# SeonghwanSeo/PharmacoNet

Hardware: AMD Instinct MI355X
Metric: ligand-conformers scored/sec (1 pocket) (higher is better)
Workload: dtype f32; 1 GPU; 6OIM-like model (37 nodes, 11 clusters) vs 1003520 synthetic ligands per GPU = 4096 molecule topologies x 245 copies with every node displaced (sigma 0.35 A) and every conformer coordinate jittered (sigma 0.30 A); mean 17.1 pharmacophore nodes (<= 32), 8 conformers each, 10 % drawn on the model's nodes; top-1000; library=expanded, pockets=1, ligands_per_gpu=1003520, conformers_per_ligand=8, parallelism=single GPU

## Files before the change

### include/pmx.h

```cpp
#ifndef PMX_H
#define PMX_H

#include <stdint.h>

#ifdef __cplusplus
extern "C" {
#endif

#define PMX_NUM_TYPES 7
#define PMX_MAX_LEVELS 20
#define PMX_MAX_MODEL_NODES 256
#define PMX_MAX_MODEL_CLUSTERS 128
#define PMX_MAX_LEVEL_CANDIDATES 64
#define PMX_MAX_LIGAND_NODES 64
#define PMX_MAX_LIGAND_CLUSTERS 64
#define PMX_MAX_CONFORMERS 64

typedef enum {
    PMX_OK = 0,
    PMX_ERR_INVALID = 1,
    PMX_ERR_HIP = 2,
    PMX_ERR_OOM = 3
} pmx_status;

// ... 73 lines not shown
    const uint64_t *atom_off;
    const uint8_t *atomic_num;
    const uint64_t *nbr_off;
    const int32_t *nbr;
    const uint64_t *feat_off;
    const uint8_t *feat_type;
    const uint8_t *feat_flags;
    const uint64_t *feat_atom_off;
    const int32_t *feat_atoms;
    const uint64_t *feat_center_off;
    const int32_t *feat_centers;
    const int32_t *n_conf;
    const uint64_t *pos_off;
    const float *positions;
} pmx_feature_batch;
int pmx_pack_features(const pmx_feature_batch *batch, int threads, uint64_t *offsets_out, uint8_t *data_out, uint64_t data_cap,
                      uint64_t *data_bytes, int32_t *status_out);
int pmx_pack_features_device(const pmx_feature_batch *batch, int device, void *stream, uint64_t *offsets_out, uint8_t *data_out,
                             uint64_t data_cap, uint64_t *data_bytes, int32_t *status_out);

int pmx_library_select(const pmx_library *lib, const uint64_t *indices_dev, uint64_t n, uint64_t *offsets_out_dev ,
                       uint8_t *data_out_dev, uint64_t data_cap, uint64_t *data_bytes, void *stream);
int pmx_library_buffers(const pmx_library *lib, const uint64_t **offsets_dev, const uint8_t **data_dev);

typedef struct {
    uint64_t n_mols;
    const uint64_t *atom_off;
    const uint8_t *atomic_num;
    const uint8_t *explicit_degree;
    const uint8_t *heavy_degree;
    const uint8_t *hyb;
    const uint8_t *h_count;
    const uint8_t *flags;
    const uint64_t *nbr_off;
    const int32_t *nbr;
    const uint64_t *ring_off;
    const uint64_t *ring_atom_off;
    const int32_t *ring_atoms;
} pmx_atom_batch;
int pmx_perceive_features(const pmx_atom_batch *batch, int threads, uint64_t *feat_off, uint8_t *feat_type, uint8_t *feat_flags,
                          uint64_t *feat_atom_off, int32_t *feat_atoms, uint64_t *feat_center_off, int32_t *feat_centers,
                          uint64_t cap_features, uint64_t cap_atoms, uint64_t cap_centers, uint64_t *n_features, uint64_t *n_feat_atoms,
                          uint64_t *n_feat_centers, int32_t *status_out);

int pmx_sdf_heavy_atoms(const char *text, uint64_t len, uint64_t max_records, uint64_t cap_records, uint64_t cap_atoms,
                        uint64_t *n_records, uint64_t *n_atoms, int32_t *atoms_per_record, uint8_t *atomic_num, float *xyz);
// ... 90 lines not shown
```

### pharmaconet_amd/_ffi.py

```python

from __future__ import annotations

import ctypes
from pathlib import Path

PKG = Path(__file__).resolve().parent
LIB_PATH = PKG / "libpmx.so"

NUM_TYPES = 7
COMM_ID_BYTES = 128


class PmxError(RuntimeError):
    pass


class ModelDesc(ctypes.Structure):
    _fields_ = [
        ("n_nodes", ctypes.c_int32),
        ("n_clusters", ctypes.c_int32),
        ("node_type", ctypes.c_void_p),
        ("edge_mean", ctypes.c_void_p),
        ("edge_std", ctypes.c_void_p),
        ("cluster_nodes", ctypes.c_void_p),
# ... 67 lines not shown

class MatchConstraint(ctypes.Structure):

    _fields_ = [
        ("n_require", ctypes.c_int32),
        ("require", (ctypes.c_uint64 * 2) * MAX_REQUIRE_GROUPS),
        ("exclude", ctypes.c_uint64 * 2),
    ]


SIGNATURES = {
    "pmx_last_error": (ctypes.c_char_p, []),
    "pmx_version": (ctypes.c_int, []),
    "pmx_model_create": (ctypes.c_int, [ctypes.POINTER(ModelDesc), ctypes.c_int, ctypes.POINTER(ctypes.c_void_p)]),
    "pmx_model_destroy": (ctypes.c_int, [ctypes.c_void_p]),
    "pmx_library_upload": (ctypes.c_int, [ctypes.POINTER(LibraryView), ctypes.c_int, ctypes.POINTER(ctypes.c_void_p)]),
    "pmx_library_info_get": (ctypes.c_int, [ctypes.c_void_p, ctypes.POINTER(LibraryInfo)]),
    "pmx_library_destroy": (ctypes.c_int, [ctypes.c_void_p]),
    "pmx_library_select": (
        ctypes.c_int,
        [ctypes.c_void_p, ctypes.c_void_p, ctypes.c_uint64, ctypes.c_void_p, ctypes.c_void_p, ctypes.c_uint64, ctypes.POINTER(ctypes.c_uint64), ctypes.c_void_p],
    ),
    "pmx_library_buffers": (ctypes.c_int, [ctypes.c_void_p, ctypes.POINTER(ctypes.c_void_p), ctypes.POINTER(ctypes.c_void_p)]),
    "pmx_score": (
        ctypes.c_int,
        [ctypes.c_void_p, ctypes.c_void_p, ctypes.POINTER(ctypes.c_float), ctypes.c_uint64, ctypes.c_uint64,
         ctypes.c_void_p, ctypes.c_void_p, ctypes.c_void_p],
    ),
    "pmx_score_multi": (
        ctypes.c_int,
        [ctypes.POINTER(ctypes.c_void_p), ctypes.c_int, ctypes.c_void_p, ctypes.POINTER(ctypes.c_float),
         ctypes.c_uint64, ctypes.c_uint64, ctypes.c_void_p, ctypes.c_void_p, ctypes.c_void_p],
    ),
    "pmx_score_f64": (
        ctypes.c_int,
        [ctypes.c_void_p, ctypes.c_void_p, ctypes.POINTER(ctypes.c_float), ctypes.c_uint64, ctypes.c_uint64,
         ctypes.c_void_p, ctypes.c_void_p, ctypes.c_void_p],
    ),
    "pmx_score_multi_f64": (
        ctypes.c_int,
        [ctypes.POINTER(ctypes.c_void_p), ctypes.c_int, ctypes.c_void_p, ctypes.POINTER(ctypes.c_float),
         ctypes.c_uint64, ctypes.c_uint64, ctypes.c_void_p, ctypes.c_void_p, ctypes.c_void_p],
    ),
    "pmx_topk": (
        ctypes.c_int,
        [ctypes.c_void_p, ctypes.c_void_p, ctypes.c_uint64, ctypes.c_uint64, ctypes.c_int, ctypes.c_void_p,
# ... 133 lines not shown
```

### pharmaconet_amd/build.py

```python

from __future__ import annotations

import os
import shutil
import subprocess
import sys
from pathlib import Path

PKG = Path(__file__).resolve().parent
REPO = PKG.parent
CSRC = PKG / "csrc"
LIB = PKG / "libpmx.so"
PACK_LIB = PKG / "libpmx_pack.so"
SOURCES = ("pmx_api.hip", "pmx_screen_debug.hip", "pmx_explain.hip", "pmx_rows.hip", "pmx_fingerprint.hip", "pmx_topk.hip", "pmx_density.hip", "pmx_pack_device.hip", "pmx_select.hip", "pmx_pack.cpp", "pmx_sdf.cpp", "pmx_perceive.cpp")
DEPS = ("pmx_screen.hip", "pmx_screen_walk.h", "pmx_screen_tables.h", "pmx_screen_layout.h", "pmx_device.h", "pmx_debug.h", "pmx_explain.h", "pmx_rows.h", "pmx_scan.h")
FLAGS = (
    "--offload-arch=gfx950",
    "-O3",
    "-std=c++17",
    "-fPIC",
    "-ffp-contract=off",
    "-fno-fast-math",
    "-Wall",
    "-Wno-unused-function",
    "-mllvm", "-simplifycfg-sink-common=false",
    "-mllvm", "-disable-lsr",
    "-mllvm", "-greedy-regclass-priority-trumps-globalness",
    "-mllvm", "-phi-node-folding-threshold=1",
)


def hipcc() -> str:
    for cand in (os.environ.get("HIPCC"), shutil.which("hipcc"), "/opt/rocm/bin/hipcc"):
        if cand and Path(cand).exists():
            return cand
    raise RuntimeError("hipcc not found")


# ... 97 lines not shown
```

### pharmaconet_amd/csrc/pmx_api.hip

```cpp
#include <hip/hip_runtime.h>

#include <algorithm>
#include <cmath>
#include <cstdarg>
#include <cstdio>
#include <cstdlib>
#include <chrono>
#include <cstring>
#include <cstddef>
#include <memory>
#include <map>
#include <mutex>
#include <string>
#include <thread>
#include <utility>
#include <vector>
#include <time.h>

#include "pmx.h"
#include "pmx_screen.hip"
#include "pmx_debug.h"
#include "pmx_explain.h"
#include "pmx_rows.h"

using namespace pmx;

static thread_local char g_err[512] = "";
static thread_local pmx_score_stats g_stats = {};
static int g_profiling = 0;
struct ScreenWs;
static thread_local std::shared_ptr<ScreenWs> g_last_screen;
static thread_local int g_last_device = 0;
static int screen_stats(pmx_score_stats *out);

static int fail(int code, const char *fmt, ...) {
    va_list ap;
    va_start(ap, fmt);
    vsnprintf(g_err, sizeof(g_err), fmt, ap);
    va_end(ap);
    return code;
}

#define HIPCHECK(expr)                                                                                         \
    do {                                                                                                       \
        hipError_t e_ = (expr);                                                                                \
// ... 456 lines not shown
    lib->info.n_bytes = nbytes;
    lib->info.total_conformers = stats[0];
    lib->info.max_nodes = (int32_t)stats[1];
    lib->info.max_conformers = (int32_t)stats[2];
    lib->info.max_clusters = (int32_t)stats[3];
    lib->info.n_unsupported = (int32_t)stats[4];
    *out = lib;
    return PMX_OK;
}

extern "C" int pmx_library_info_get(const pmx_library *lib, pmx_library_info *info) {
    if (!lib || !info) return fail(PMX_ERR_INVALID, "null argument");
    *info = lib->info;
    return PMX_OK;
}

extern "C" int pmx_library_buffers(const pmx_library *lib, const uint64_t **offsets_dev, const uint8_t **data_dev) {
    if (!lib || !offsets_dev || !data_dev) return fail(PMX_ERR_INVALID, "null argument");
    *offsets_dev = lib->offsets;
    *data_dev = lib->data;
    return PMX_OK;
}

int pmx_library_device(const pmx_library *lib) { return lib->device; }

extern "C" int pmx_library_destroy(pmx_library *lib) {
    if (!lib) return PMX_OK;
    (void)hipSetDevice(lib->device);
    if (lib->owns) (void)hipFree(lib->offsets), (void)hipFree(lib->data);
    delete lib;
    return PMX_OK;
}

static std::mutex g_mu;

static long env_long(const char *name, long dflt) {
    const char *s = std::getenv(name);
    if (!s || !*s) return dflt;
    return std::atol(s);
}

static constexpr size_t kLdsPerCu = 160 * 1024;

static bool trace_on() {
    static int v = -1;
    if (v < 0) v = std::getenv("PMX_TRACE") ? 1 : 0;
    return v == 1;
}

struct ScreenWs {
    DevBuf ctl;
    DevBuf xctl;
    DevBuf slices, big;
    DevBuf totbuf;
    DevBuf pabuf;
    DevBuf arena, queue;
    DevBuf lists;
    DevBuf acur;
    size_t arena_shrunk_to = 0;
    int num_cu = 0;
    hipEvent_t ev[6] = {nullptr, nullptr, nullptr, nullptr, nullptr, nullptr};
    uint64_t ligands_last = 0;
    bool ev_valid = false;
    bool ctl_used = false;
    hipStream_t last_stream = nullptr;
    std::mutex mu;
    uint64_t stamp = 0;
    bool released = false;
    void free_buffers() {
        for (DevBuf *b : {&ctl, &xctl, &slices, &big, &totbuf, &pabuf, &arena, &queue, &lists, &acur}) b->release();
        for (auto &e : ev) {
            if (e) (void)hipEventDestroy(e);
            e = nullptr;
        }
        arena_shrunk_to = 0;
        ev_valid = ctl_used = false;
    }
};
static std::map<std::pair<int, hipStream_t>, std::shared_ptr<ScreenWs>> g_screen;

static uint64_t g_screen_stamp = 0;

static std::shared_ptr<ScreenWs> ensure_screen(int device, hipStream_t stream) {
    std::shared_ptr<ScreenWs> out, victim;
    {
        std::lock_guard<std::mutex> lock(g_mu);
        const auto key = std::make_pair(device, stream);
        auto it = g_screen.find(key);
        if (it != g_screen.end() && it->second) {
            it->second->stamp = ++g_screen_stamp;
            return it->second;
        }
        const long cap = std::max<long>(1, env_long("PMX_MAX_WORKSPACES", 4));
// ... 142 lines not shown
    pl.need.big = (size_t)pl.big_grid * pl.big_bytes;
    if (cand_bounds<G>()) {
        const uint64_t need = (nlmax + 1) * nlmax * K * G * 4;
        p.pa_bytes = (uint32_t)std::min<uint64_t>((need + 255) & ~255ull, (uint64_t)std::max<long>(1, env_long("PMX_PATH_KB", 1024)) << 10);
        pl.need.pabuf = (size_t)grid * p.pa_bytes * 2u;
    }
    if (!totals_in_lds<G>()) pl.need.totbuf = (size_t)num_cu * 4u * std::max(PMX_SCREEN_WAVES, PMX_TASK_WAVES) * kTotBufBytes * 2u;
    if (worst > pl.big_bytes) pl.arena_retries = (int)std::max<long>(1, env_long("PMX_ARENA_RETRIES", 4));
    const long super_dflt = std::max(16384L, (1L << 20) * 8 / std::max(G, 8) / k_scale);
    pl.super = (uint32_t)std::max<long>(1024, std::min<long>(env_long("PMX_SUPER", super_dflt), 1 << 24));
    return PMX_OK;
}

template <int G>
static int score_screen(const pmx_model *const *models, int n_models, const pmx_library *lib, const Weights &W, uint64_t first, uint64_t count,
                        void *scores_dev, bool scores_f64, int32_t *status_dev, hipStream_t stream, ScreenWs &ws) {
    if (count > 0xfffffff0ull) return fail(PMX_ERR_INVALID, "more than 2^32 ligands in one call");
    const uint32_t flags = (uint32_t)env_long("PMX_TREE_FLAGS", 0);
    const uint32_t lig_budget = (uint32_t)std::max<long>(16, env_long("PMX_BUDGET", 768));
    const uint32_t task_budget = (uint32_t)std::max<long>(16, env_long("PMX_TASK_BUDGET", std::min<long>(lig_budget, 384)));
    const int rounds = (int)std::max<long>(1, env_long("PMX_ROUNDS", 12));
    const int task_decay_from = (int)std::max<long>(1, env_long("PMX_TASK_DECAY_FROM", 99));
    const uint32_t task_budget_min = (uint32_t)std::max<long>(8, env_long("PMX_TASK_BUDGET_MIN", 48));
    const bool exact = (flags & 8) != 0;
    const bool debug_kernels = (flags & ~PMX_PRODUCT_FLAGS) != 0;
    bool debug_ok = true;
    const bool tails = pair_tails(models, n_models, W);

    {
        const int irc = init_workspace(ws, lib->device, stream);
        if (irc) return irc;
    }
    std::vector<PocketPlan> plan((size_t)n_models);
    BufferNeeds need;
    uint32_t super_max = 0;
    for (int m = 0; m < n_models; ++m) {
        PocketPlan &pl = plan[(size_t)m];
        const int rc = plan_pocket<G>(models[m], lib, W, ws.num_cu, stream, pl);
        if (rc) return rc;
        ScreenParams &p = pl.p;
        p.first = first;
        p.flags = flags | (scores_f64 ? PMX_SCORES_F64 : 0u);
        p.budget = lig_budget;
        p.min_levels = (uint32_t)std::max<long>(0, env_long("PMX_MIN_LEVELS", 3));
        p.scores = scores_f64 ? reinterpret_cast<float *>(static_cast<double *>(scores_dev) + (size_t)m * count) : static_cast<float *>(scores_dev) + (size_t)m * count;
        p.status = m == 0 ? status_dev : nullptr;
        need.cover(pl.need);
        super_max = std::max(super_max, pl.super);
    }

    {
        int rc = grow_buffers(ws, need, stream);
        if (!rc) rc = ensure_arena<G>(ws, stream);
        if (rc) return rc;
        HIPCHECK(ws.queue.grow((size_t)std::max<long>(1, env_long("PMX_TASKQ_MB", (G >= 32 ? 1024L : 2048L) * std::max(1, G / 8))) << 20, stream));
        HIPCHECK(ws.lists.grow((size_t)super_max * 12, stream));
    }
    Ctl *const ctl = ws.ctl.as<Ctl>();
    uint32_t *const lists = ws.lists.as<uint32_t>();
    uint8_t *const totbuf = ws.totbuf.as<uint8_t>(), *const pabuf = ws.pabuf.as<uint8_t>();

    if (g_profiling) HIPCHECK(hipEventRecord(ws.ev[0], stream));
    ws.ctl_used = false;
    for (int m = 0; m < n_models; ++m) {
        const PocketPlan &pl = plan[(size_t)m];
        ScreenParams p = pl.p;
        const uint32_t super = pl.super;
        const uint32_t lig_grid = (uint32_t)ws.num_cu * pl.waves_per_cu, task_grid = (uint32_t)ws.num_cu * pl.task_waves_per_cu;
        p.ctl = ctl;
        p.arena = ws.arena.as<uint8_t>();
        p.arena_bytes = std::min<unsigned long long>(ws.arena.bytes, (1ull << 36) - 4096);
        p.ovf_list = lists;
        p.carry_list = lists + super;
        p.heavy_list = lists + 2 * (size_t)super;
        p.list_cap = super;
        p.queue = ws.queue.as<uint8_t>();
        p.qcap = (uint32_t)std::min<size_t>(ws.queue.bytes / task_rec_bytes<G>() / kShards, 0x3fffffffu / kShards);
        p.totbuf = totbuf;
        p.pabuf = pabuf;
        auto launch = [&](int mode, uint32_t blocks) {
            p.mode = mode;
            if (debug_kernels) debug_ok &= pmx_debug::launch_ligand(G, exact, tails, blocks, pl.lds, stream, &p, sizeof p);
            else if (tails) ligand_kernel<G, false, true><<<dim3(blocks), dim3(64), pl.lds, stream>>>(p);
            else ligand_kernel<G, false, false><<<dim3(blocks), dim3(64), pl.lds, stream>>>(p);
        };
        auto rounds_and_finalize = [&]() {
            if (!totals_in_lds<G>()) p.totbuf = totbuf + ws.totbuf.bytes / 2;
            if (pabuf) p.pabuf = pabuf + ws.pabuf.bytes / 2;
            for (int r = 0; r < rounds; ++r) {
                p.budget = r < task_decay_from ? task_budget : std::max<uint32_t>(task_budget_min, task_budget >> std::min(r - task_decay_from + 1, 16));
                p.last_round = r + 1 == rounds ? 1u : 0u;
                round_kernel<<<dim3(1), dim3(64), 0, stream>>>(ctl, p.qcap);
                if (debug_kernels) debug_ok &= pmx_debug::launch_task(G, task_grid, pl.lds, stream, &p, sizeof p);
                else task_kernel<G><<<dim3(task_grid), dim3(64), pl.lds, stream>>>(p);
            }
            finalize_kernel<G><<<dim3((super + 255) / 256), dim3(256), 0, stream>>>(p);
            p.last_round = 0;
            p.budget = lig_budget;
            p.totbuf = totbuf;
            p.pabuf = pabuf;
        };
        for (uint64_t lo = 0; lo < count; lo += super) {
            const bool last_of_call = m + 1 == n_models && lo + super >= count;
            p.lo = (uint32_t)lo;
            p.hi = (uint32_t)std::min<uint64_t>(count, lo + super);
            if (g_profiling && last_of_call) HIPCHECK(hipEventRecord(ws.ev[1], stream));
            ws.ligands_last = p.hi - p.lo;
            ctl_clear_kernel<<<dim3((sizeof(Ctl) / 4 + 255) / 256), dim3(256), 0, stream>>>(ctl, ws.ctl_used ? 0 : 1);
            ws.ctl_used = true;
            p.slices = ws.slices.as<uint8_t>();
            p.slice_bytes = pl.slice_bytes;
            launch(0, lig_grid);
            p.slices = ws.big.as<uint8_t>();
            p.slice_bytes = pl.big_bytes;
            launch(1, std::min(pl.big_grid, lig_grid));
            p.retry_out = lists;
            p.retry_slot = 0;
            launch(2, std::min(pl.big_grid, lig_grid));
            if (g_profiling && last_of_call) {
                HIPCHECK(hipEventRecord(ws.ev[2], stream));
                HIPCHECK(hipEventRecord(ws.ev[4], stream));
            }
            rounds_and_finalize();
            for (int t = 0; t < pl.arena_retries; ++t) {
                prepare_retry(p, ctl, lists, super, t, pl.arena_retries, stream);
                launch(3, std::min(pl.big_grid, lig_grid));
                rounds_and_finalize();
            }
// ... 60 lines not shown

static int lanes_of(const pmx_library *lib) {
    int g = 1;
    while (g < std::min(lib->info.max_conformers, PMX_MAX_CONFORMERS)) g <<= 1;
    return g;
}

static Weights to_weights(const float weights[PMX_NUM_TYPES]) {
    Weights W;
    for (int t = 0; t < PMX_NUM_TYPES; ++t) W.w[t] = weights[t];
    return W;
}

struct HeldWs {
    std::shared_ptr<ScreenWs> ws;
    std::unique_lock<std::mutex> lock;
};
static HeldWs hold_screen(int device, hipStream_t stream) {
    for (;;) {
        HeldWs h{ensure_screen(device, stream), {}};
        h.lock = std::unique_lock<std::mutex>(h.ws->mu);
        if (!h.ws->released) return h;
    }
}

static int score_any(const pmx_model *const *models, int n_models, const pmx_library *lib, const float weights[PMX_NUM_TYPES], uint64_t first,
                     uint64_t count, void *scores_dev, bool scores_f64, int32_t *status_dev, void *stream_) {
    if (!models || n_models < 0 || !lib || !weights || (!scores_dev && count && n_models)) return fail(PMX_ERR_INVALID, "null argument");
    for (int i = 0; i < n_models; ++i) {
        if (!models[i]) return fail(PMX_ERR_INVALID, "null model");
        if (models[i]->device != lib->device) return fail(PMX_ERR_INVALID, "model and library live on different devices");
    }
    if (first > lib->info.n_ligands || count > lib->info.n_ligands - first) return fail(PMX_ERR_INVALID, "ligand range out of bounds");
    g_stats = pmx_score_stats{};
    g_last_screen.reset();
    if (count == 0 || n_models == 0) return PMX_OK;
    HIPCHECK(hipSetDevice(lib->device));
    const Weights W = to_weights(weights);
    hipStream_t stream = static_cast<hipStream_t>(stream_);
    const HeldWs held = hold_screen(lib->device, stream);
    int rc = PMX_OK;
    if (!with_lanes(lanes_of(lib), [&](auto g) { rc = score_screen<decltype(g)::value>(models, n_models, lib, W, first, count, scores_dev, scores_f64, status_dev, stream, *held.ws); }))
        rc = fail(PMX_ERR_INVALID, "no kernels for %d conformer lanes", lanes_of(lib));
    g_last_screen = held.ws;
    g_last_device = lib->device;
    return rc;
// ... 234 lines not shown
```

### pharmaconet_amd/csrc/pmx_debug.h

```cpp
#pragma once
#include <hip/hip_runtime.h>
#include <cstddef>

namespace pmx_debug {
bool launch_ligand(int G, bool exact, bool tails, unsigned blocks, unsigned lds, hipStream_t stream, const void *params, size_t bytes);
bool launch_task(int G, unsigned blocks, unsigned lds, hipStream_t stream, const void *params, size_t bytes);
}
```

### pharmaconet_amd/csrc/pmx_screen.hip

```cpp
#include "pmx_screen_walk.h"

#ifndef PMX_SCREEN_WAVES
#define PMX_SCREEN_WAVES 6
#endif
#ifndef PMX_TASK_WAVES
#define PMX_TASK_WAVES 6
#endif

namespace PMX_NS {
using namespace pmx;

template <int G, bool EXACT, bool TAILS>
__global__ __launch_bounds__(64, PMX_SCREEN_WAVES) void ligand_kernel(const ScreenParams p) {
    extern __shared__ __attribute__((aligned(16))) unsigned char lds[];
    const int lane0 = lane_id();
    const uint32_t wave_id = blockIdx.x;
    const WaveShape<G> ws = wave_shape<G>(p.M.K, (int)p.max_nodes);
    const uint32_t todo = p.mode == 0 ? p.hi - p.lo
                          : min(p.mode == 1 ? p.ctl->ovf_count : (p.mode == 2 ? p.ctl->carry_count : p.ctl->retry_count[p.retry_slot ^ 1u]), p.list_cap);
    const uint32_t *list = p.mode == 1 ? p.ovf_list : (p.mode == 2 ? p.carry_list : p.retry_in);
    constexpr uint32_t kBatch = 1;
    WaveStats *stat = reinterpret_cast<WaveStats *>(lds + ws.off_stat);
    if (lane0 < (int)(sizeof(WaveStats) / 8)) reinterpret_cast<unsigned long long *>(stat)[lane0] = 0ull;
    wave_sync();
    const unsigned long long t_start = __builtin_amdgcn_s_memtime();
    uint32_t lig_next = 0, lig_end = 0;
    for (;;) {
        const int lane = lane_id();
        if (lig_next == lig_end) {
            uint32_t base = 0;
            if (lane == 0) base = atomicAdd(&p.ctl->cursor[p.mode], kBatch);
            base = (uint32_t)uni((int)base);
            lig_next = min(base, todo);
            lig_end = min(base + kBatch, todo);
            if (lig_next == lig_end) break;
        }
        const uint32_t next = lig_next++;
        const uint32_t li = p.mode == 0 ? p.lo + next : (uint32_t)uni((int)list[next]);
        unsigned char *rec = prepare_ligand<G, EXACT, TAILS>(p, lds, ws, li, wave_id, stat);
        if (!rec) continue;
        const unsigned char *root = lds + ws.off_task;
        const uint32_t rec16 = (uint32_t)uni((int)reinterpret_cast<const TaskRec *>(root)->rec16);
        Walk<G> w;
        if (!(PMX_WFLAGS(p) & 16384) && prepare_walk<G>(p, lds, ws, root, rec, w)) run_job<G>(p, lds, ws, w, rec, rec16, false, wave_id, stat);
    }
    wave_sync();
    if (lane0 == 0) flush_wave_stats(p, stat, wave_id, __builtin_amdgcn_s_memtime() - t_start);
}

__global__ void round_kernel(Ctl *ctl, uint32_t qcap) {
    const int lane = threadIdx.x & 63;
    const uint32_t lo = ctl->round_hi[lane], hi = min(ctl->q_res[lane], qcap);
    uint32_t n = hi - lo, inc = n;
#pragma unroll
    for (int d = 1; d < 64; d <<= 1) {
        const uint32_t t = __shfl_up(inc, d);
        if (lane >= d) inc += t;
    }
#pragma unroll
    for (int d = 1; d < 64; d <<= 1) n += __shfl_xor(n, d);
    ctl->round_lo[lane] = lo;
    ctl->round_hi[lane] = hi;
    ctl->round_inc[lane] = inc;
    if (lane == 0) {
        ctl->round_total = n;
        ctl->task_cursor = 0;
        for (int x = 0; x < 8; ++x) ctl->xcd_cursor[x][0] = 0;
// ... 19 lines not shown
        uint32_t nx = 0xffffffffu;
        while (skip < 8) {
            const int xx = (int)((blockIdx.x + skip) & 7u);
            const uint32_t st = xx ? (uint32_t)rl((int)inc, 8 * xx - 1) : 0u, en = (uint32_t)rl((int)inc, 8 * xx + 7);
            if (st < en) {
                uint32_t cur = 0;
                if (lane == 0) cur = atomicAdd(&p.ctl->xcd_cursor[xx][0], 1u);
                cur = (uint32_t)uni((int)cur);
                if (cur < en - st) {
                    nx = st + cur;
                    break;
                }
            }
            ++skip;
        }
        if (nx == 0xffffffffu) break;
        const int sh = __popcll(__ballot(nx >= inc));
        const uint32_t before = sh ? (uint32_t)rl((int)inc, sh - 1) : 0u;
        const uint32_t recno = (uint32_t)uni((int)p.ctl->round_lo[sh]) + (nx - before);
        const unsigned char *tr = p.queue + ((size_t)sh * p.qcap + recno) * task_rec_bytes<G>();
        if (lane == 0) ++stat->tasks;
        unsigned char *rec = p.arena + (size_t)(uint32_t)uni((int)reinterpret_cast<const TaskRec *>(tr)->rec16) * 16;
        Walk<G> w;
        if (prepare_walk<G>(p, lds, ws, tr, rec, w)) run_job<G>(p, lds, ws, w, rec, (uint32_t)((rec - p.arena) >> 4), true, wave_id, stat);
    }
    wave_sync();
    if (lane0 == 0) flush_wave_stats(p, stat, wave_id, __builtin_amdgcn_s_memtime() - t_start);
}

template <int G>
__global__ void finalize_kernel(const ScreenParams p) {
    const uint32_t i = blockIdx.x * blockDim.x + threadIdx.x;
    if (i >= min(p.ctl->heavy_count, p.list_cap)) return;
    const unsigned char *rec = p.arena + (size_t)p.heavy_list[i] * 16;
    const RecHeader *H = reinterpret_cast<const RecHeader *>(rec);
    const unsigned long long *best = reinterpret_cast<const unsigned long long *>(rec + sizeof(RecHeader));
    const int C = (int)H->C;
    double sum = 0.0;
    for (int c = 0; c < C; ++c) sum += __longlong_as_double((long long)best[c]);
    put_score(p, H->lig, sum / (double)C);
}

__global__ void retry_prep_kernel(Ctl *ctl, uint32_t slot_out) {
    const int lane = threadIdx.x & 63;
    ctl->q_res[lane] = 0;
    ctl->round_lo[lane] = 0;
    ctl->round_hi[lane] = 0;
// ... 88 lines not shown
```

### pharmaconet_amd/csrc/pmx_screen_debug.hip

```cpp
#include <hip/hip_runtime.h>
#include <cstring>

#define PMX_DEBUG_KERNELS 1
#define PMX_NS pmx_dbg
#include "pmx_screen.hip"
#include "pmx_debug.h"

namespace pmx_debug {

bool launch_ligand(int G, bool exact, bool tails, unsigned blocks, unsigned lds, hipStream_t stream, const void *params, size_t bytes) {
    if (bytes != sizeof(pmx_dbg::ScreenParams)) return false;
    pmx_dbg::ScreenParams p;
    std::memcpy(&p, params, sizeof p);
    return pmx::with_lanes(G, [&](auto g) {
        constexpr int L = decltype(g)::value;
        if (exact) pmx_dbg::ligand_kernel<L, true, false><<<dim3(blocks), dim3(64), lds, stream>>>(p);
        else if (tails) pmx_dbg::ligand_kernel<L, false, true><<<dim3(blocks), dim3(64), lds, stream>>>(p);
        else pmx_dbg::ligand_kernel<L, false, false><<<dim3(blocks), dim3(64), lds, stream>>>(p);
    });
}

bool launch_task(int G, unsigned blocks, unsigned lds, hipStream_t stream, const void *params, size_t bytes) {
    if (bytes != sizeof(pmx_dbg::ScreenParams)) return false;
    pmx_dbg::ScreenParams p;
    std::memcpy(&p, params, sizeof p);
    return pmx::with_lanes(G, [&](auto g) { pmx_dbg::task_kernel<decltype(g)::value><<<dim3(blocks), dim3(64), lds, stream>>>(p); });
}

}
```

### pharmaconet_amd/csrc/pmx_screen_layout.h

```cpp
#pragma once
#include "pmx_device.h"

#pragma clang fp contract(off)

#ifndef PMX_NS
#define PMX_NS pmx
#endif
#define PMX_SCORES_F64 (1u << 30)
#define PMX_PRODUCT_FLAGS (2u | 16384u)
#ifdef PMX_DEBUG_KERNELS
#define PMX_WFLAGS(p) ((p).flags)
#else
#define PMX_WFLAGS(p) ((p).flags & PMX_PRODUCT_FLAGS)
#endif

#ifndef PMX_TC_LEVELS
#define PMX_TC_LEVELS 4
#endif

namespace PMX_NS {
using namespace pmx;

struct FnCell {
    float c[6];
// ... 144 lines not shown
    uint8_t *slices;
    uint32_t slice_bytes;
    uint8_t *arena;
    unsigned long long arena_bytes;
    uint32_t *ovf_list, *carry_list, *heavy_list;
    uint32_t list_cap;
    uint8_t *queue;
    uint32_t qcap;
    uint32_t budget;
    uint32_t min_levels;
    uint32_t flags;
    uint32_t max_nodes;
    uint32_t last_round;
    uint32_t bound_cost;
    uint32_t dead_min_entries;
    float *scores;
    int32_t *status;
    int mode;
    const uint32_t *retry_in;
    uint32_t *retry_out;
    uint32_t retry_slot;
};

constexpr int kTcLevels = PMX_TC_LEVELS;
static_assert(kTcLevels >= 1 && kTcLevels <= 8, "cache slot number is three bits of Walk::hk");
template <int G>
struct WaveShape {
    uint32_t kp;
    uint32_t nc_cap;
    uint32_t off_cand, off_lcnt, off_nc, off_tot, off_pool, off_stat, off_task, off_tch, off_tc, off_cb, off_ub, bytes;
};
template <int G>
__host__ __device__ inline WaveShape<G> wave_shape(int K, int max_nodes) {
    WaveShape<G> w;
    w.kp = (uint32_t)((K + 3) & ~3);
    w.nc_cap = w.kp * (uint32_t)((max_nodes + 3) & ~3);
    uint32_t o = 512;
    w.off_cand = o;
    o += PMX_MAX_LEVELS * w.kp;
    w.off_lcnt = o;
    o += PMX_MAX_LEVELS * w.kp;
    o = (o + 15u) & ~15u;
    w.off_nc = o;
    o += w.nc_cap * 2;
    o = (o + 15u) & ~15u;
    w.off_tot = o;
// ... 27 lines not shown
```

### pharmaconet_amd/csrc/pmx_screen_walk.h

```cpp
#pragma once
#include "pmx_screen_tables.h"

#ifndef PMX_ROW_BATCH
#define PMX_ROW_BATCH 8
#endif
#ifndef PMX_PATH_WINDOWS
#define PMX_PATH_WINDOWS 3
#endif
#ifndef PMX_PATH_MIN_LEVELS
#define PMX_PATH_MIN_LEVELS 3
#endif
#ifndef PMX_SHARE_EVERY
#define PMX_SHARE_EVERY 16
#endif

namespace PMX_NS {
using namespace pmx;


template <int G>
struct Walk {
    const unsigned char *Sb, *Pb, *Rb, *Wb, *Vb, *OBb;
    int nl;
    uint32_t ksumtot;
// ... 775 lines not shown
    if (s == 0) {
        tot[nm0 * G + c] = reinterpret_cast<const double *>(tr + sizeof(TaskRec))[c];
        pool[c] = __hip_atomic_load(&gbest[c], __ATOMIC_RELAXED, __HIP_MEMORY_SCOPE_AGENT);
    }
    w.f = w.f0 = f0;
    const uint64_t mask0 = uni64(th->mask);
    w.stA = wl(w.stA, f0, (int)(uint32_t)mask0);
    if (G > 32) w.stB = wl(w.stB, f0, (int)(uint32_t)(mask0 >> 32));
    else w.stB = -1;
    w.stC = wl(w.stC, f0, (((nm0 ? (int)kMatched : 0) | (w.path_on ? (int)kPath : 0)) << 16) | (nm0 << 24));
    wave_sync();
    if (!(PMX_WFLAGS(p) & 4) && f0 < nl && nm0 >= 5) {
        const double r = *reinterpret_cast<const double *>(w.Rb + ((size_t)f0 * G + c) * 8);
        const double t = tot[nm0 * G + c];
        if (__ballot(((mask0 >> c) & 1ull) && (t + r) * kBoundSlack > __longlong_as_double((long long)pool[c])) == 0) return false;
    }
    if (cand_bounds<G>() && w.path_on && nm0 > 0)
        path_sums_of_root<G>(w, reinterpret_cast<float *>(p.pabuf + (size_t)blockIdx.x * p.pa_bytes), nm0);
    return true;
}

template <int G>
__device__ __forceinline__ void run_job(const ScreenParams &p, unsigned char *lds, const WaveShape<G> &ws, Walk<G> &w, unsigned char *rec, uint32_t rec16,
                                        const bool is_task, const uint32_t wave_id, WaveStats *stat) {
    const int lane = lane_id();
    const int s = lane / G, c = lane % G;
    double *tot = totals_in_lds<G>() ? reinterpret_cast<double *>(lds + ws.off_tot) : reinterpret_cast<double *>(p.totbuf + (size_t)blockIdx.x * kTotBufBytes);
    unsigned long long *pool = reinterpret_cast<unsigned long long *>(lds + ws.off_pool);
    uint16_t *pathbuf = reinterpret_cast<uint16_t *>(lds + kOffPath);
    double *tch = reinterpret_cast<double *>(lds + ws.off_tch);
    double *tc = reinterpret_cast<double *>(lds + ws.off_tc);
    unsigned long long *cbl = reinterpret_cast<unsigned long long *>(lds + ws.off_cb);
    float *pa = reinterpret_cast<float *>(p.pabuf + (size_t)blockIdx.x * p.pa_bytes);
    float *ub = reinterpret_cast<float *>(lds + ws.off_ub);
    const unsigned long long t_d = __builtin_amdgcn_s_memtime();
    unsigned long long budget = ((PMX_WFLAGS(p) & 2) || p.last_round) ? ~0ull : (unsigned long long)p.budget;
    bool export_mode = false, split = is_task;
    for (;;) {
        const int rc = walk<G>(w, p, tot, pool, pathbuf, tch, tc, cbl, pa, ub, rec16, export_mode, budget, wave_id, stat);
        if (rc != kOverBudget) break;
        if (lane == 0) ++stat->over;
        budget = ~0ull;
        RecHeader *H = reinterpret_cast<RecHeader *>(rec);
        if (rec16 == 0) {
            const uint32_t bytes = (uint32_t)uni((int)H->bytes);
            const unsigned long long off = arena_alloc(p, bytes);
            if (off != ~0ull) {
                const uint4 *src = reinterpret_cast<const uint4 *>(rec);
                uint4 *dst = reinterpret_cast<uint4 *>(p.arena + off);
                const uint32_t n16 = (bytes + 15u) / 16u;
                for (uint32_t i = lane; i < n16; i += 64) dst[i] = src[i];
                rec16 = (uint32_t)(off >> 4);
                rec = p.arena + off;
            }
        }
        if (rec16 != 0) {
            export_mode = true;
            H = reinterpret_cast<RecHeader *>(rec);
            if (!is_task && !split) {
// ... 35 lines not shown
```

### pharmaconet_amd/engine.py

```python

from __future__ import annotations

import contextlib
import ctypes
from dataclasses import dataclass

import numpy as np

from . import _ffi
from .constants import weights_vector
from .library import PackedLibrary, as_packed_library

__all__ = ["Alignment", "Attribution", "DeviceLibrary", "Explanation", "PanelResult", "ScreeningResult", "align", "attribute", "explain", "score_one", "screen", "screen_multi", "topk",
           "device_model", "last_score_stats"]


def _torch():
    import torch

    if not torch.cuda.is_available():
        raise _ffi.PmxError("no GPU visible: pharmaconet_amd scores on an MI355X only (there is no CPU path)")
    return torch


# ... 105 lines not shown
            raise _ffi.PmxError("a molecule exceeds the device packer's fixed scratch (include/pmx.h): use library.pack_features_native for this batch")
        self = cls.from_device_buffers(offsets, data, device if device is not None else offsets.device, adopt=True)
        self.pack_status = status
        return self

    def __len__(self) -> int:
        return self.num_ligands

    def select(self, indices) -> "DeviceLibrary":
        torch = _torch()
        lib = _ffi.load()
        tdev = torch.device("cuda", self.device)
        idx = _listed_indices(indices, tdev)
        n = int(idx.numel())
        with torch.cuda.device(tdev):
            stream = ctypes.c_void_p(torch.cuda.current_stream(tdev).cuda_stream)
            offsets = torch.empty(n + 1, dtype=torch.int64, device=tdev)
            nbytes = ctypes.c_uint64(0)
            _ffi.check(lib.pmx_library_select(self.handle, idx.data_ptr() if n else None, n, offsets.data_ptr(), None, 0, ctypes.byref(nbytes), stream))
            data = torch.empty(int(nbytes.value), dtype=torch.uint8, device=tdev)
            if data.numel():
                _ffi.check(lib.pmx_library_select(self.handle, idx.data_ptr(), n, offsets.data_ptr(), data.data_ptr(), data.numel(), ctypes.byref(nbytes), stream))
            return DeviceLibrary.from_device_buffers(offsets, data, tdev, adopt=True)

    def buffers(self):
        src = getattr(self, "_adopted", None)
        if src is not None:
            return src
        torch = _torch()
        po, pd = ctypes.c_void_p(), ctypes.c_void_p()
        _ffi.check(_ffi.load().pmx_library_buffers(self.handle, ctypes.byref(po), ctypes.byref(pd)))
        tdev = torch.device("cuda", self.device)

        class _View:
            def __init__(self, ptr, count, typestr):
                self.__cuda_array_interface__ = dict(shape=(count,), typestr=typestr, data=(int(ptr), False), version=2, strides=None)

        offsets = torch.as_tensor(_View(po.value, self.num_ligands + 1, "<i8"), device=tdev)
        data = torch.as_tensor(_View(pd.value, self.num_bytes, "|u1"), device=tdev) if self.num_bytes else torch.empty(0, dtype=torch.uint8, device=tdev)
        return offsets, data

    def download(self) -> PackedLibrary:
        offsets, data = self.buffers()
        return PackedLibrary(offsets.cpu().numpy().view(np.uint64).copy(), data[: self.num_bytes].cpu().numpy().copy())

    def close(self) -> None:
# ... 906 lines not shown
```

### pharmaconet_amd/library.py

```python

from __future__ import annotations

import struct
from collections.abc import Iterable, Sequence
from dataclasses import dataclass, field
from pathlib import Path

import numpy as np

from .constants import (
    CLUSTER_PRIORITY,
    MAX_CONFORMERS,
    MAX_LIGAND_CLUSTERS,
    MAX_LIGAND_NODES,
    TYPE_ID,
)

__all__ = [
    "LigandFeatures",
    "ClusteredLigand",
    "PackedLibrary",
    "cluster_ligand",
    "pack_clustered_ligand",
    "record_node_atoms",
# ... 283 lines not shown
    status = np.zeros(n, dtype=np.int32)
    nbytes = ctypes.c_uint64(0)
    def check(rc):
        if rc != 0:
            raise _ffi.PmxError(f"libpmx_pack error {rc}: {lib.pmx_last_error().decode()}")

    check(lib.pmx_pack_features(ctypes.byref(batch), int(threads), offsets.ctypes.data, None, 0, ctypes.byref(nbytes), status.ctypes.data))
    data = np.empty(int(nbytes.value), dtype=np.uint8)
    check(lib.pmx_pack_features(ctypes.byref(batch), int(threads), offsets.ctypes.data, data.ctypes.data, data.size, ctypes.byref(nbytes),
                                status.ctypes.data))
    return PackedLibrary(offsets, data[: int(nbytes.value)]), status


UNSUPPORTED_RECORD = _HEADER.pack(0, 0, 0, 0) + b"\0" * (RECORD_ALIGN - _HEADER.size)


def pack_ligand_or_marker(lig: LigandFeatures) -> tuple[bytes, str | None]:
    try:
        return pack_ligand(lig), None
    except LigandTooLarge as e:
        return UNSUPPORTED_RECORD, str(e)


@dataclass
class PackedLibrary:
    offsets: np.ndarray
    data: np.ndarray

    def __len__(self) -> int:
        return int(self.offsets.shape[0]) - 1

    @classmethod
    def from_records(cls, records: Sequence[bytes]) -> "PackedLibrary":
        sizes = np.fromiter((len(r) for r in records), dtype=np.uint64, count=len(records))
        if np.any(sizes % RECORD_ALIGN):
            raise ValueError("records must be padded to 16 bytes")
        offsets = np.zeros(len(records) + 1, dtype=np.uint64)
        np.cumsum(sizes, out=offsets[1:])
        data = np.frombuffer(b"".join(records), dtype=np.uint8).copy()
        return cls(offsets, data)

    def record(self, i: int) -> bytes:
        return self.data[int(self.offsets[i]) : int(self.offsets[i + 1])].tobytes()

    def header(self, i: int) -> tuple[int, int, int]:
        n, c, k, _ = _HEADER.unpack_from(self.data, int(self.offsets[i]))
        return n, c, k

    def headers(self) -> np.ndarray:
        starts = self.offsets[:-1].astype(np.int64)
        raw = self.data
        out = np.empty((len(self), 3), dtype=np.uint16)
        for col in range(3):
            lo = raw[starts + 2 * col].astype(np.uint16)
            hi = raw[starts + 2 * col + 1].astype(np.uint16)
            out[:, col] = lo | (hi << 8)
        return out

    def num_conformers(self) -> np.ndarray:
        return self.headers()[:, 1].astype(np.int64)

    def slice(self, first: int, count: int) -> "PackedLibrary":
        lo, hi = int(self.offsets[first]), int(self.offsets[first + count])
        return PackedLibrary(self.offsets[first : first + count + 1] - np.uint64(lo), self.data[lo:hi])

    def select(self, indices) -> "PackedLibrary":
        idx = np.asarray(indices, dtype=np.int64).reshape(-1)
        if idx.size and (int(idx.min()) < 0 or int(idx.max()) >= len(self)):
            bad = np.flatnonzero((idx < 0) | (idx >= len(self)))
            raise IndexError(f"{len(bad)} of {len(idx)} indices are outside the library's {len(self)} ligands, the first at position {int(bad[0])}")
        data = np.ascontiguousarray(self.data[: int(self.offsets[-1])])
        if np.any(self.offsets % RECORD_ALIGN):
            raise ValueError("records must start on 16-byte boundaries")
        starts = self.offsets[idx].astype(np.int64) // RECORD_ALIGN
        sizes = self.offsets[idx + 1].astype(np.int64) // RECORD_ALIGN - starts
        ends = np.cumsum(sizes)
        offsets = np.zeros(len(idx) + 1, dtype=np.uint64)
        offsets[1:] = ends * RECORD_ALIGN
        src = np.repeat(starts - (ends - sizes), sizes) + np.arange(int(ends[-1]) if len(idx) else 0, dtype=np.int64)
        return PackedLibrary(offsets, data.view(f"V{RECORD_ALIGN}")[src].view(np.uint8))

    def unpack(self, i: int) -> dict:
        n, c, k = self.header(i)
# ... 47 lines not shown
```

Measured before the change: 88.22 million ligand-conformers/s.

## Claim ligands heaviest-first via device radix-sorted order to reduce tail imbalance

Adds a device pass that builds a per-super-batch ligand order with a hipcub radix sort, keyed so ligands with more clusters and nodes come first. The persistent ligand kernel then claims ligands in that order, so long jobs start early and short ones fill the tail, reducing load imbalance at the end of each batch. It also adds an optional walk budget that scales with the remaining work, but that is off by default (slope 0). The cost is an extra key kernel and sort per batch, more scattered record access, and one more indirection per claimed ligand.

```diff
diff --git a/include/pmx.h b/include/pmx.h
--- a/include/pmx.h
+++ b/include/pmx.h
@@ -119,6 +119,8 @@
 int pmx_library_select(const pmx_library *lib, const uint64_t *indices_dev, uint64_t n, uint64_t *offsets_out_dev ,
                        uint8_t *data_out_dev, uint64_t data_cap, uint64_t *data_bytes, void *stream);
 int pmx_library_buffers(const pmx_library *lib, const uint64_t **offsets_dev, const uint8_t **data_dev);
+int pmx_library_order(const pmx_library *lib, uint64_t lo, uint64_t hi, uint32_t *out_dev, void *stream);
+uint32_t pmx_library_order_key(uint32_t n_nodes, uint32_t n_conformers, uint32_t n_clusters);
 
 typedef struct {
     uint64_t n_mols;
diff --git a/pharmaconet_amd/_ffi.py b/pharmaconet_amd/_ffi.py
--- a/pharmaconet_amd/_ffi.py
+++ b/pharmaconet_amd/_ffi.py
@@ -113,6 +113,8 @@
         [ctypes.c_void_p, ctypes.c_void_p, ctypes.c_uint64, ctypes.c_void_p, ctypes.c_void_p, ctypes.c_uint64, ctypes.POINTER(ctypes.c_uint64), ctypes.c_void_p],
     ),
     "pmx_library_buffers": (ctypes.c_int, [ctypes.c_void_p, ctypes.POINTER(ctypes.c_void_p), ctypes.POINTER(ctypes.c_void_p)]),
+    "pmx_library_order": (ctypes.c_int, [ctypes.c_void_p, ctypes.c_uint64, ctypes.c_uint64, ctypes.c_void_p, ctypes.c_void_p]),
+    "pmx_library_order_key": (ctypes.c_uint32, [ctypes.c_uint32, ctypes.c_uint32, ctypes.c_uint32]),
     "pmx_score": (
         ctypes.c_int,
         [ctypes.c_void_p, ctypes.c_void_p, ctypes.POINTER(ctypes.c_float), ctypes.c_uint64, ctypes.c_uint64,
diff --git a/pharmaconet_amd/build.py b/pharmaconet_amd/build.py
--- a/pharmaconet_amd/build.py
+++ b/pharmaconet_amd/build.py
@@ -12,8 +12,8 @@
 CSRC = PKG / "csrc"
 LIB = PKG / "libpmx.so"
 PACK_LIB = PKG / "libpmx_pack.so"
-SOURCES = ("pmx_api.hip", "pmx_screen_debug.hip", "pmx_explain.hip", "pmx_rows.hip", "pmx_fingerprint.hip", "pmx_topk.hip", "pmx_density.hip", "pmx_pack_device.hip", "pmx_select.hip", "pmx_pack.cpp", "pmx_sdf.cpp", "pmx_perceive.cpp")
-DEPS = ("pmx_screen.hip", "pmx_screen_walk.h", "pmx_screen_tables.h", "pmx_screen_layout.h", "pmx_device.h", "pmx_debug.h", "pmx_explain.h", "pmx_rows.h", "pmx_scan.h")
+SOURCES = ("pmx_api.hip", "pmx_screen_debug.hip", "pmx_explain.hip", "pmx_rows.hip", "pmx_fingerprint.hip", "pmx_topk.hip", "pmx_density.hip", "pmx_pack_device.hip", "pmx_select.hip", "pmx_order.hip", "pmx_pack.cpp", "pmx_sdf.cpp", "pmx_perceive.cpp")
+DEPS = ("pmx_screen.hip", "pmx_screen_walk.h", "pmx_screen_tables.h", "pmx_screen_layout.h", "pmx_device.h", "pmx_debug.h", "pmx_explain.h", "pmx_rows.h", "pmx_scan.h", "pmx_order.h")
 FLAGS = (
     "--offload-arch=gfx950",
     "-O3",
diff --git a/pharmaconet_amd/csrc/pmx_api.hip b/pharmaconet_amd/csrc/pmx_api.hip
--- a/pharmaconet_amd/csrc/pmx_api.hip
+++ b/pharmaconet_amd/csrc/pmx_api.hip
@@ -21,6 +21,7 @@
 #include "pmx_screen.hip"
 #include "pmx_debug.h"
 #include "pmx_explain.h"
+#include "pmx_order.h"
 #include "pmx_rows.h"
 
 using namespace pmx;
@@ -523,6 +524,18 @@
     return PMX_OK;
 }
 
+static int library_order(const pmx_library *lib, uint64_t lo, uint64_t hi, uint32_t *out_dev, hipStream_t stream);
+extern "C" int pmx_library_order(const pmx_library *lib, uint64_t lo, uint64_t hi, uint32_t *out_dev, void *stream) {
+    if (!lib) return fail(PMX_ERR_INVALID, "null argument");
+    if (lo > hi || hi > lib->info.n_ligands) return fail(PMX_ERR_INVALID, "ligand range out of bounds");
+    if (hi > 0xffffffffull || hi - lo > 0x7fffffffull) return fail(PMX_ERR_INVALID, "pmx_library_order: indices beyond 2^32 or more than 2^31 - 1 ligands in one call");
+    if (lo == hi) return PMX_OK;
+    if (!out_dev) return fail(PMX_ERR_INVALID, "null argument");
+    return library_order(lib, lo, hi, out_dev, static_cast<hipStream_t>(stream));
+}
+
+extern "C" uint32_t pmx_library_order_key(uint32_t n_nodes, uint32_t n_conformers, uint32_t n_clusters) { return pmx_order::order_key(n_nodes, n_conformers, n_clusters); }
+
 int pmx_library_device(const pmx_library *lib) { return lib->device; }
 
 extern "C" int pmx_library_destroy(pmx_library *lib) {
@@ -542,6 +555,7 @@
 }
 
 static constexpr size_t kLdsPerCu = 160 * 1024;
+static constexpr long kOrderDefault = 1, kBudgetSlopeDefault = 0;
 
 static bool trace_on() {
     static int v = -1;
@@ -558,6 +572,8 @@
     DevBuf arena, queue;
     DevBuf lists;
     DevBuf acur;
+    DevBuf order;
+    pmx_order::Work order_work;
     size_t arena_shrunk_to = 0;
     int num_cu = 0;
     hipEvent_t ev[6] = {nullptr, nullptr, nullptr, nullptr, nullptr, nullptr};
@@ -569,7 +585,8 @@
     uint64_t stamp = 0;
     bool released = false;
     void free_buffers() {
-        for (DevBuf *b : {&ctl, &xctl, &slices, &big, &totbuf, &pabuf, &arena, &queue, &lists, &acur}) b->release();
+        for (DevBuf *b : {&ctl, &xctl, &slices, &big, &totbuf, &pabuf, &arena, &queue, &lists, &acur, &order}) b->release();
+        order_work.release();
         for (auto &e : ev) {
             if (e) (void)hipEventDestroy(e);
             e = nullptr;
@@ -758,6 +775,8 @@
     const int rounds = (int)std::max<long>(1, env_long("PMX_ROUNDS", 12));
     const int task_decay_from = (int)std::max<long>(1, env_long("PMX_TASK_DECAY_FROM", 99));
     const uint32_t task_budget_min = (uint32_t)std::max<long>(8, env_long("PMX_TASK_BUDGET_MIN", 48));
+    const bool use_order = env_long("PMX_ORDER", kOrderDefault) != 0;
+    const long budget_slope = std::max<long>(0, std::min<long>(env_long("PMX_BUDGET_SLOPE", kBudgetSlopeDefault), 1L << 30));
     const bool exact = (flags & 8) != 0;
     const bool debug_kernels = (flags & ~PMX_PRODUCT_FLAGS) != 0;
     bool debug_ok = true;
@@ -791,7 +810,9 @@
         if (rc) return rc;
         HIPCHECK(ws.queue.grow((size_t)std::max<long>(1, env_long("PMX_TASKQ_MB", (G >= 32 ? 1024L : 2048L) * std::max(1, G / 8))) << 20, stream));
         HIPCHECK(ws.lists.grow((size_t)super_max * 12, stream));
-    }
+        if (use_order) HIPCHECK(ws.order.grow((size_t)count * 4, stream));
+    }
+    uint32_t order_super = 0;
     Ctl *const ctl = ws.ctl.as<Ctl>();
     uint32_t *const lists = ws.lists.as<uint32_t>();
     uint8_t *const totbuf = ws.totbuf.as<uint8_t>(), *const pabuf = ws.pabuf.as<uint8_t>();
@@ -814,11 +835,19 @@
         p.qcap = (uint32_t)std::min<size_t>(ws.queue.bytes / task_rec_bytes<G>() / kShards, 0x3fffffffu / kShards);
         p.totbuf = totbuf;
         p.pabuf = pabuf;
+        ClaimParams cp{nullptr, (float)((double)budget_slope / (double)lig_grid), 0u};
+        if (use_order && order_super != super) {
+            for (uint64_t lo = 0; lo < count; lo += super) {
+                const uint32_t n = (uint32_t)std::min<uint64_t>(super, count - lo);
+                HIPCHECK(pmx_order::build(p.lib, first + lo, n, (uint32_t)lo, ws.order.as<uint32_t>() + lo, ws.order_work, stream));
+            }
+            order_super = super;
+        }
         auto launch = [&](int mode, uint32_t blocks) {
             p.mode = mode;
-            if (debug_kernels) debug_ok &= pmx_debug::launch_ligand(G, exact, tails, blocks, pl.lds, stream, &p, sizeof p);
-            else if (tails) ligand_kernel<G, false, true><<<dim3(blocks), dim3(64), pl.lds, stream>>>(p);
-            else ligand_kernel<G, false, false><<<dim3(blocks), dim3(64), pl.lds, stream>>>(p);
+            if (debug_kernels) debug_ok &= pmx_debug::launch_ligand(G, exact, tails, blocks, pl.lds, stream, &p, sizeof p, &cp, sizeof cp);
+            else if (tails) ligand_kernel<G, false, true><<<dim3(blocks), dim3(64), pl.lds, stream>>>(p, cp);
+            else ligand_kernel<G, false, false><<<dim3(blocks), dim3(64), pl.lds, stream>>>(p, cp);
         };
         auto rounds_and_finalize = [&]() {
             if (!totals_in_lds<G>()) p.totbuf = totbuf + ws.totbuf.bytes / 2;
@@ -840,6 +869,7 @@
             const bool last_of_call = m + 1 == n_models && lo + super >= count;
             p.lo = (uint32_t)lo;
             p.hi = (uint32_t)std::min<uint64_t>(count, lo + super);
+            cp.order = use_order ? ws.order.as<uint32_t>() + lo : nullptr;
             if (g_profiling && last_of_call) HIPCHECK(hipEventRecord(ws.ev[1], stream));
             ws.ligands_last = p.hi - p.lo;
             ctl_clear_kernel<<<dim3((sizeof(Ctl) / 4 + 255) / 256), dim3(256), 0, stream>>>(ctl, ws.ctl_used ? 0 : 1);
@@ -946,6 +976,13 @@
         h.lock = std::unique_lock<std::mutex>(h.ws->mu);
         if (!h.ws->released) return h;
     }
+}
+
+static int library_order(const pmx_library *lib, uint64_t lo, uint64_t hi, uint32_t *out_dev, hipStream_t stream) {
+    HIPCHECK(hipSetDevice(lib->device));
+    const HeldWs held = hold_screen(lib->device, stream);
+    HIPCHECK(pmx_order::build(lib->dl, lo, (uint32_t)(hi - lo), (uint32_t)lo, out_dev, held.ws->order_work, stream));
+    return PMX_OK;
 }
 
 static int score_any(const pmx_model *const *models, int n_models, const pmx_library *lib, const float weights[PMX_NUM_TYPES], uint64_t first,
diff --git a/pharmaconet_amd/csrc/pmx_debug.h b/pharmaconet_amd/csrc/pmx_debug.h
--- a/pharmaconet_amd/csrc/pmx_debug.h
+++ b/pharmaconet_amd/csrc/pmx_debug.h
@@ -3,6 +3,6 @@
 #include <cstddef>
 
 namespace pmx_debug {
-bool launch_ligand(int G, bool exact, bool tails, unsigned blocks, unsigned lds, hipStream_t stream, const void *params, size_t bytes);
+bool launch_ligand(int G, bool exact, bool tails, unsigned blocks, unsigned lds, hipStream_t stream, const void *params, size_t bytes, const void *claim, size_t claim_bytes);
 bool launch_task(int G, unsigned blocks, unsigned lds, hipStream_t stream, const void *params, size_t bytes);
 }
diff --git a/pharmaconet_amd/csrc/pmx_order.h b/pharmaconet_amd/csrc/pmx_order.h
--- /dev/null
+++ b/pharmaconet_amd/csrc/pmx_order.h
@@ -0,0 +1,23 @@
+#pragma once
+#include "pmx_device.h"
+
+namespace pmx_order {
+
+constexpr uint32_t kKeyBits = 14;
+constexpr uint32_t kLast = (1u << kKeyBits) - 1u;
+__host__ __device__ inline uint32_t order_key(uint32_t n_nodes, uint32_t n_conf, uint32_t n_clusters) {
+    const bool scored = n_conf >= 1 && n_conf <= PMX_MAX_CONFORMERS && n_nodes <= PMX_MAX_LIGAND_NODES && n_clusters <= PMX_MAX_LIGAND_CLUSTERS;
+    return scored ? ((uint32_t)(PMX_MAX_LIGAND_CLUSTERS - n_clusters) << 7) | (uint32_t)(PMX_MAX_LIGAND_NODES - n_nodes) : kLast;
+}
+static_assert(PMX_MAX_LIGAND_CLUSTERS <= 64 && PMX_MAX_LIGAND_NODES <= 64, "two 7-bit fields, and kLast above every scored key");
+
+struct Work {
+    pmx::DevBuf keys, vals, scratch;
+    void release() {
+        for (pmx::DevBuf *b : {&keys, &vals, &scratch}) b->release();
+    }
+};
+
+hipError_t build(const pmx::DevLibrary &lib, uint64_t lib_first, uint32_t n, uint32_t value_base, uint32_t *out, Work &w, hipStream_t stream);
+
+}
diff --git a/pharmaconet_amd/csrc/pmx_order.hip b/pharmaconet_amd/csrc/pmx_order.hip
--- /dev/null
+++ b/pharmaconet_amd/csrc/pmx_order.hip
@@ -0,0 +1,39 @@
+#include <hip/hip_runtime.h>
+#include <hipcub/hipcub.hpp>
+
+#include <cstdint>
+
+#include "pmx_order.h"
+
+namespace pmx_order {
+namespace {
+
+__global__ __launch_bounds__(256) void key_kernel(pmx::DevLibrary lib, uint64_t lib_first, uint32_t n, uint32_t value_base, uint32_t *keys, uint32_t *vals) {
+    const uint32_t i = blockIdx.x * 256u + threadIdx.x;
+    if (i >= n) return;
+    const uint64_t h = *reinterpret_cast<const uint64_t *>(lib.data + lib.offsets[lib_first + i]);
+    keys[i] = order_key((uint32_t)(h & 0xffffu), (uint32_t)(h >> 16 & 0xffffu), (uint32_t)(h >> 32 & 0xffffu));
+    vals[i] = value_base + i;
+}
+
+}
+
+hipError_t build(const pmx::DevLibrary &lib, uint64_t lib_first, uint32_t n, uint32_t value_base, uint32_t *out, Work &w, hipStream_t stream) {
+    if (n == 0) return hipSuccess;
+    if (n > 0x7fffffffu) return hipErrorInvalidValue;
+    size_t scratch_need = 0;
+    hipError_t e = hipcub::DeviceRadixSort::SortPairs(nullptr, scratch_need, (const uint32_t *)nullptr, (uint32_t *)nullptr, (const uint32_t *)nullptr, (uint32_t *)nullptr,
+                                                      (int)n, 0, (int)kKeyBits, stream);
+    if (e == hipSuccess) e = w.keys.grow((size_t)n * 8, stream);
+    if (e == hipSuccess) e = w.vals.grow((size_t)n * 4, stream);
+    if (e == hipSuccess) e = w.scratch.grow(scratch_need ? scratch_need : 8, stream);
+    if (e != hipSuccess) return e;
+    uint32_t *keys = w.keys.as<uint32_t>(), *vals = w.vals.as<uint32_t>();
+    key_kernel<<<dim3((n + 255u) / 256u), dim3(256), 0, stream>>>(lib, lib_first, n, value_base, keys, vals);
+    e = hipGetLastError();
+    if (e != hipSuccess) return e;
+    size_t scratch_bytes = w.scratch.bytes;
+    return hipcub::DeviceRadixSort::SortPairs(w.scratch.ptr, scratch_bytes, keys, keys + n, vals, out, (int)n, 0, (int)kKeyBits, stream);
+}
+
+}
diff --git a/pharmaconet_amd/csrc/pmx_screen.hip b/pharmaconet_amd/csrc/pmx_screen.hip
--- a/pharmaconet_amd/csrc/pmx_screen.hip
+++ b/pharmaconet_amd/csrc/pmx_screen.hip
@@ -11,7 +11,7 @@
 using namespace pmx;
 
 template <int G, bool EXACT, bool TAILS>
-__global__ __launch_bounds__(64, PMX_SCREEN_WAVES) void ligand_kernel(const ScreenParams p) {
+__global__ __launch_bounds__(64, PMX_SCREEN_WAVES) void ligand_kernel(const ScreenParams p, const ClaimParams cp) {
     extern __shared__ __attribute__((aligned(16))) unsigned char lds[];
     const int lane0 = lane_id();
     const uint32_t wave_id = blockIdx.x;
@@ -36,13 +36,15 @@
             if (lig_next == lig_end) break;
         }
         const uint32_t next = lig_next++;
-        const uint32_t li = p.mode == 0 ? p.lo + next : (uint32_t)uni((int)list[next]);
+        const uint32_t li = p.mode == 0 ? (cp.order ? (uint32_t)uni((int)cp.order[next]) : p.lo + next) : (uint32_t)uni((int)list[next]);
         unsigned char *rec = prepare_ligand<G, EXACT, TAILS>(p, lds, ws, li, wave_id, stat);
         if (!rec) continue;
         const unsigned char *root = lds + ws.off_task;
         const uint32_t rec16 = (uint32_t)uni((int)reinterpret_cast<const TaskRec *>(root)->rec16);
         Walk<G> w;
-        if (!(PMX_WFLAGS(p) & 16384) && prepare_walk<G>(p, lds, ws, root, rec, w)) run_job<G>(p, lds, ws, w, rec, rec16, false, wave_id, stat);
+        uint32_t budget = p.budget;
+        if (p.mode == 0) budget = max(budget, (uint32_t)uni((int)(uint32_t)fminf((float)(todo - lig_next + 1u) * cp.budget_slope, 4.0e9f)));
+        if (!(PMX_WFLAGS(p) & 16384) && prepare_walk<G>(p, lds, ws, root, rec, w)) run_job<G>(p, lds, ws, w, rec, rec16, false, budget, wave_id, stat);
     }
     wave_sync();
     if (lane0 == 0) flush_wave_stats(p, stat, wave_id, __builtin_amdgcn_s_memtime() - t_start);
@@ -108,7 +110,7 @@
         if (lane == 0) ++stat->tasks;
         unsigned char *rec = p.arena + (size_t)(uint32_t)uni((int)reinterpret_cast<const TaskRec *>(tr)->rec16) * 16;
         Walk<G> w;
-        if (prepare_walk<G>(p, lds, ws, tr, rec, w)) run_job<G>(p, lds, ws, w, rec, (uint32_t)((rec - p.arena) >> 4), true, wave_id, stat);
+        if (prepare_walk<G>(p, lds, ws, tr, rec, w)) run_job<G>(p, lds, ws, w, rec, (uint32_t)((rec - p.arena) >> 4), true, p.budget, wave_id, stat);
     }
     wave_sync();
     if (lane0 == 0) flush_wave_stats(p, stat, wave_id, __builtin_amdgcn_s_memtime() - t_start);
diff --git a/pharmaconet_amd/csrc/pmx_screen_debug.hip b/pharmaconet_amd/csrc/pmx_screen_debug.hip
--- a/pharmaconet_amd/csrc/pmx_screen_debug.hip
+++ b/pharmaconet_amd/csrc/pmx_screen_debug.hip
@@ -8,15 +8,17 @@
 
 namespace pmx_debug {
 
-bool launch_ligand(int G, bool exact, bool tails, unsigned blocks, unsigned lds, hipStream_t stream, const void *params, size_t bytes) {
-    if (bytes != sizeof(pmx_dbg::ScreenParams)) return false;
+bool launch_ligand(int G, bool exact, bool tails, unsigned blocks, unsigned lds, hipStream_t stream, const void *params, size_t bytes, const void *claim, size_t claim_bytes) {
+    if (bytes != sizeof(pmx_dbg::ScreenParams) || claim_bytes != sizeof(pmx_dbg::ClaimParams)) return false;
     pmx_dbg::ScreenParams p;
     std::memcpy(&p, params, sizeof p);
+    pmx_dbg::ClaimParams cp;
+    std::memcpy(&cp, claim, sizeof cp);
     return pmx::with_lanes(G, [&](auto g) {
         constexpr int L = decltype(g)::value;
-        if (exact) pmx_dbg::ligand_kernel<L, true, false><<<dim3(blocks), dim3(64), lds, stream>>>(p);
-        else if (tails) pmx_dbg::ligand_kernel<L, false, true><<<dim3(blocks), dim3(64), lds, stream>>>(p);
-        else pmx_dbg::ligand_kernel<L, false, false><<<dim3(blocks), dim3(64), lds, stream>>>(p);
+        if (exact) pmx_dbg::ligand_kernel<L, true, false><<<dim3(blocks), dim3(64), lds, stream>>>(p, cp);
+        else if (tails) pmx_dbg::ligand_kernel<L, false, true><<<dim3(blocks), dim3(64), lds, stream>>>(p, cp);
+        else pmx_dbg::ligand_kernel<L, false, false><<<dim3(blocks), dim3(64), lds, stream>>>(p, cp);
     });
 }
 
diff --git a/pharmaconet_amd/csrc/pmx_screen_layout.h b/pharmaconet_amd/csrc/pmx_screen_layout.h
--- a/pharmaconet_amd/csrc/pmx_screen_layout.h
+++ b/pharmaconet_amd/csrc/pmx_screen_layout.h
@@ -190,6 +190,12 @@
     uint32_t retry_slot;
 };
 
+struct ClaimParams {
+    const uint32_t *order;
+    float budget_slope;
+    uint32_t pad_;
+};
+
 constexpr int kTcLevels = PMX_TC_LEVELS;
 static_assert(kTcLevels >= 1 && kTcLevels <= 8, "cache slot number is three bits of Walk::hk");
 template <int G>
diff --git a/pharmaconet_amd/csrc/pmx_screen_walk.h b/pharmaconet_amd/csrc/pmx_screen_walk.h
--- a/pharmaconet_amd/csrc/pmx_screen_walk.h
+++ b/pharmaconet_amd/csrc/pmx_screen_walk.h
@@ -821,7 +821,7 @@
 
 template <int G>
 __device__ __forceinline__ void run_job(const ScreenParams &p, unsigned char *lds, const WaveShape<G> &ws, Walk<G> &w, unsigned char *rec, uint32_t rec16,
-                                        const bool is_task, const uint32_t wave_id, WaveStats *stat) {
+                                        const bool is_task, const uint32_t walk_budget, const uint32_t wave_id, WaveStats *stat) {
     const int lane = lane_id();
     const int s = lane / G, c = lane % G;
     double *tot = totals_in_lds<G>() ? reinterpret_cast<double *>(lds + ws.off_tot) : reinterpret_cast<double *>(p.totbuf + (size_t)blockIdx.x * kTotBufBytes);
@@ -833,7 +833,7 @@
     float *pa = reinterpret_cast<float *>(p.pabuf + (size_t)blockIdx.x * p.pa_bytes);
     float *ub = reinterpret_cast<float *>(lds + ws.off_ub);
     const unsigned long long t_d = __builtin_amdgcn_s_memtime();
-    unsigned long long budget = ((PMX_WFLAGS(p) & 2) || p.last_round) ? ~0ull : (unsigned long long)p.budget;
+    unsigned long long budget = ((PMX_WFLAGS(p) & 2) || p.last_round) ? ~0ull : (unsigned long long)walk_budget;
     bool export_mode = false, split = is_task;
     for (;;) {
         const int rc = walk<G>(w, p, tot, pool, pathbuf, tch, tc, cbl, pa, ub, rec16, export_mode, budget, wave_id, stat);
diff --git a/pharmaconet_amd/engine.py b/pharmaconet_amd/engine.py
--- a/pharmaconet_amd/engine.py
+++ b/pharmaconet_amd/engine.py
@@ -151,6 +151,16 @@
             if data.numel():
                 _ffi.check(lib.pmx_library_select(self.handle, idx.data_ptr(), n, offsets.data_ptr(), data.data_ptr(), data.numel(), ctypes.byref(nbytes), stream))
             return DeviceLibrary.from_device_buffers(offsets, data, tdev, adopt=True)
+
+    def order(self, lo: int = 0, hi: int | None = None):
+        torch = _torch()
+        tdev = torch.device("cuda", self.device)
+        hi = self.num_ligands if hi is None else hi
+        with torch.cuda.device(tdev):
+            out = torch.empty(max(hi - lo, 0), dtype=torch.int32, device=tdev)
+            stream = ctypes.c_void_p(torch.cuda.current_stream(tdev).cuda_stream)
+            _ffi.check(_ffi.load().pmx_library_order(self.handle, lo, hi, out.data_ptr() if out.numel() else None, stream))
+            return out.to(torch.int64)
 
     def buffers(self):
         src = getattr(self, "_adopted", None)
diff --git a/pharmaconet_amd/library.py b/pharmaconet_amd/library.py
--- a/pharmaconet_amd/library.py
+++ b/pharmaconet_amd/library.py
@@ -329,6 +329,18 @@
         return UNSUPPORTED_RECORD, str(e)
 
 
+MAX_LIGAND_NODES = MAX_LIGAND_CLUSTERS = MAX_CONFORMERS = 64
+ORDER_KEY_BITS = 14
+ORDER_KEY_LAST = (1 << ORDER_KEY_BITS) - 1
+
+
+def order_key(headers: np.ndarray) -> np.ndarray:
+    h = np.asarray(headers, dtype=np.int64).reshape(-1, 3)
+    n, c, k = h[:, 0], h[:, 1], h[:, 2]
+    scored = (c >= 1) & (c <= MAX_CONFORMERS) & (n <= MAX_LIGAND_NODES) & (k <= MAX_LIGAND_CLUSTERS)
+    return np.where(scored, ((MAX_LIGAND_CLUSTERS - k) << 7) | (MAX_LIGAND_NODES - n), ORDER_KEY_LAST).astype(np.uint32)
+
+
 @dataclass
 class PackedLibrary:
     offsets: np.ndarray
@@ -366,6 +378,10 @@
 
     def num_conformers(self) -> np.ndarray:
         return self.headers()[:, 1].astype(np.int64)
+
+    def heavy_first(self, lo: int = 0, hi: int | None = None) -> np.ndarray:
+        hi = len(self) if hi is None else hi
+        return lo + np.argsort(order_key(self.headers()[lo:hi]), kind="stable")
 
     def slice(self, first: int, count: int) -> "PackedLibrary":
         lo, hi = int(self.offsets[first]), int(self.offsets[first + count])
```

Measured after the change: 88.16 million ligand-conformers/s. No clear change (-0.1%).
